# simonsobs/hmvec

Hardware: AMD Instinct MI355X
Metric: (z,m,k) grid-points/sec for P_1h+P_2h (higher is better)
Workload: dtype f64

## Files before the change

### hmvec_amd/_native.py

```python
import ctypes as C
import math
import os

import numpy as np

_HERE = os.path.dirname(os.path.abspath(__file__))
LIB_PATH = os.environ.get("HMG_LIB_PATH") or os.path.join(_HERE, "libhmgrid.so")
ABI_VERSION = 10
COMM_ID_BYTES = 128

c_double_p = C.c_void_p


class NativeError(RuntimeError):
    pass


class HaloStageArgs(C.Structure):
    _fields_ = [("d_zs", C.c_void_p), ("d_delta", C.c_void_p), ("d_rho", C.c_void_p),
                ("duffy_A", C.c_double), ("duffy_alpha", C.c_double), ("duffy_beta", C.c_double),
                ("h", C.c_double), ("d_cs", C.c_void_p), ("d_rvir", C.c_void_p), ("d_rs", C.c_void_p),
                ("d_nfw_series", C.c_void_p), ("d_drho1", C.c_void_p), ("delta2", C.c_double),
                ("d_rho2", C.c_void_p), ("d_m2", C.c_void_p), ("d_r2", C.c_void_p)]

# ... 109 lines not shown
    "hmg_sigma2_massfn": [_P, _I, _I, _I, _P, _P, _P, _P, _D, C.POINTER(MassFnParams), _P, _P, _P, _P, _P, _P],
    "hmg_sigma2_massfn_halo": [_P, _I, _I, _I, _P, _P, _P, _P, _D, C.POINTER(MassFnParams), _P, _P, _P, _P, _P, _P,
                               C.POINTER(HaloStageArgs)],
    "hmg_halo_stage": [_P, _I, _I, _P, _P, _P, _P, _D, _D, _D, _D, _P, _P, _P, _P, _P, _D, _P, _P, _P],
    "hmg_massfn": [_P, _I, _I, C.POINTER(MassFnParams), _P, _P, _P, _P, _P, _P],
    "hmg_halo_structure": [_P, _I, _I, _P, _P, _P, _P, _D, _D, _D, _D, _P, _P, _P],
    "hmg_mdelta_convert": [_P, _I, _I, _P, _P, _P, _D, _P, _P, _P],
    "hmg_nfw_analytic": [_P, _I, _I, _I, _P, _P, _P, _P, _P, _P],
    "hmg_profile_rowparams": [_P, _I, _I, _I, _P, _P, _P, _P, _P, _P, C.POINTER(_D * 9), _D, _D, _D,
                              _D, _P, _P, _P, _P, _P, _P, _P],
    "hmg_profile_rows_from_mvir": [_P, _I, _I, _I, _P, _P, _P, _P, _P, _D, _P, _P, C.POINTER(_D * 9), _D, _D,
                                   _D, _D, _P, _P, _P, _P, _P, _P, _P, _P, _P],
    "hmg_profile_fft": [_P, _I, _I, _I, _I, _D, _P, _P, _P, _P, _P, _P, _D, _D, _D, _D, _D,
                        _P, _P, _P, _P, _I, _P, _P, _P, _P, _P],
    "hmg_profile_fft_logx": [_P, _I, _P, _P],
    "hmg_hod": [_P, _I, _I, C.POINTER(HodParams), _P, _P, _P, _P, _P, _P, _P, _P, _P, _P, _P, _P],
    "hmg_power": [_P, _I, _I, _I, C.POINTER(Tracer), C.POINTER(Tracer), _P, _P, _P, _P, _P, _P,
                  _D, _D, _P, _P],
    "hmg_power_batch": [_P, _I, _I, _I, _I, C.POINTER(Tracer), _I, C.POINTER(_I), C.POINTER(_I),
                        _P, _P, _P, _P, _P, _P, _D, _D, C.POINTER(_P), C.POINTER(_P)],
    "hmg_power_2halo_terms": [_P, _I, _I, _I, C.POINTER(Tracer), C.POINTER(Tracer), _P, _P, _P, _P, _P, _D,
                              _P, _P, _P],
    "hmg_sigma2_halo_front": [_P, _I, _I, _I, _P, _P, _P, _P, _D, _P, C.POINTER(HaloStageArgs), C.POINTER(HodPart),
                              C.POINTER(RowsPart)],
    "hmg_group_rows": [_P, _I, _I, _I, _I, C.POINTER(MassFnPart), C.POINTER(HodPart), C.POINTER(RowsPart),
                       C.POINTER(NfwPart)],
    "hmg_group_profile": [_P, _I, _I, _I, C.POINTER(ProfileFftPart), C.POINTER(HodPart), C.POINTER(PowerBatchDesc)],
    "hmg_group_tensors": [_P, _I, _I, _I, _I, C.POINTER(MassFnPart), C.POINTER(HodPart), C.POINTER(PowerBatchDesc),
                          C.POINTER(NfwPart), C.POINTER(ProfileFftPart)],
    "hmg_power_batch_run": [_P, _I, _I, _I, C.POINTER(PowerBatchDesc), _I],
# ... 219 lines not shown
        self.call_now("hmg_event_record", slot)

    def lane(self, i):
        self.flush()
        self.call_now("hmg_lane_set", i)

    def wait(self, slot):
        self.flush()
        self.call_now("hmg_event_wait", slot)

    def elapsed_ms(self, s0, s1):
        ms = C.c_double()
        check(self.lib.hmg_elapsed_ms(self.handle, s0, s1, C.byref(ms)))
        return ms.value

    _NO_FLUSH = frozenset(["hmg_bracket_next", "hmg_profile_support_epoch"])

    def call(self, name, *args):
        if name not in self._NO_FLUSH:
            self.flush()
        if self._trace is not None:
            self._trace.append((name, args))
        check(getattr(self.lib, name)(self.handle, *args))

    def capture(self, fn):
        self.flush()
        check(self.lib.hmg_graph_begin(self.handle))
        self.capture_serial += 1
        try:
            fn()
            self.flush()
# ... 57 lines not shown
```

### hmvec_amd/csrc/hmctx.hpp

```cpp
#pragma once
#include <hip/hip_runtime.h>
#include <rccl/rccl.h>
#include <rocfft/rocfft.h>

#include <cstdio>
#include <map>
#include <string>
#include <tuple>
#include <vector>

#include "../../include/hmgrid.h"
#include "ldsfft.hpp"
#include "sici.hpp"

extern thread_local std::string g_last_error;
int fail(const char* what, const char* detail, const char* file, int line);
#define HIP_TRY(expr)                                                                   \
    do {                                                                                \
        hipError_t e_ = (expr);                                                         \
        if (e_ != hipSuccess) {                                                         \
            (void)hipGetLastError();                                                    \
            return fail(#expr, hipGetErrorString(e_), __FILE__, __LINE__);              \
        }                                                                               \
    } while (0)
// ... 38 lines not shown
    hmg::UnpackTw* twNr = nullptr;
};
struct ChirpPlan {
    hmg::cplx *chP = nullptr, *chJ = nullptr, *Bw = nullptr;
    int Jw = 0;
};
struct SupportKey {
    const void *cmax, *xs, *rss, *ks;
    int rows, nxs, nk;
    long long epoch;
    bool operator<(const SupportKey& o) const {
        return std::tie(cmax, xs, rss, ks, rows, nxs, nk, epoch) < std::tie(o.cmax, o.xs, o.rss, o.ks, o.rows, o.nxs, o.nk, o.epoch);
    }
};

struct hmg_ctx {
    int device = 0;
    hipStream_t stream = nullptr;
    hipStream_t lanes[HMG_LANES] = {};
    int lane = 0;
    hipEvent_t ev[HMG_EVENT_SLOTS] = {};
    int bracket[HMG_KERNEL_COUNT][2];
    void* scratch[7] = {nullptr, nullptr, nullptr, nullptr, nullptr, nullptr, nullptr};
    size_t scratch_bytes[7] = {0, 0, 0, 0, 0, 0, 0};
    std::map<std::pair<int, int>, FftPlan> plans;
    std::map<int, struct FusedPlan> fused;
    size_t fft_chunk_bytes = 0;
    int use_fused_fft = 1;
    int use_pruned_fft = 1;
    int fused_max_m = 6144;
// ... 22 lines not shown
    char* up_ring = nullptr;
    hipEvent_t up_ev[UP_SLOTS] = {};
    int up_next = 0;
    hipEvent_t pin_ev[2] = {nullptr, nullptr};
    int num_cu = 256;
    std::multimap<size_t, void*> free_blocks;
    std::map<void*, size_t> block_bytes;
    size_t cached_bytes = 0;
    bool lanes_dirty = false;
    bool capturing = false;
    std::vector<void*> freed_in_capture;
    std::map<int, std::vector<void*>> graph_blocks;
    std::map<int, hipGraphExec_t> graphs;
    std::map<int, int> graph_kernels;
    int next_graph_id = 1;
    hmg_ctx() { for (auto& b : bracket) b[0] = b[1] = -1; }
};
constexpr size_t FREE_CACHE_LIMIT = (size_t)4 << 30;

int event_at(hmg_ctx* c, int slot, hipEvent_t* out);
int check_fault(hmg_ctx* c);
int sync_all(hmg_ctx* c);
int ensure_scratch(hmg_ctx* c, int slot, size_t bytes);
int bracket_open(hmg_ctx* c, int kid, int* stop_slot);
int bracket_close(hmg_ctx* c, int stop_slot);
static inline dim3 grid1d(size_t n, int block) { return dim3((unsigned)((n + block - 1) / block)); }
```

### hmvec_amd/csrc/hmgrid.hip

```cpp
#include <algorithm>
#include <cmath>
#include <cstdlib>
#include <cstring>

#include "hmctx.hpp"
#include "fastmath.hpp"
#include "rowdev.hpp"
#include "longgrid.hpp"

#include "kernels/common.hpp"
#include "kernels/sigma2.hpp"
#include "kernels/massfn.hpp"
#include "kernels/halo.hpp"
#include "kernels/nfw.hpp"
#include "kernels/rows.hpp"
#include "kernels/profile_chain.hpp"
#include "kernels/profile_fused.hpp"
#include "kernels/hod.hpp"
#include "kernels/power.hpp"
#include "kernels/power_batch.hpp"
#include "kernels/groups.hpp"
#include "kernels/limber.hpp"
#include "kernels/functions.hpp"

// ... 594 lines not shown
    A.nconst = p.d_nconst; A.cconst = p.d_cconst;
    A.logx = p.d_logxs;
    A.rho_tab = R.rho_tab; A.rho_shared = R.rho_shared;
    A.rowsc = (p.d_rowsc && p.d_nconst) ? p.d_rowsc : nullptr;
    return A;
}

static int profile_fft_impl(hmg_ctx* c, int nz, int nm, int nk, const hmg_profile_fft_part& p, FftRiders& R) {
    const int nxs = p.nxs;
    const double step = p.fft_step;
    const double *xs = p.d_xs, *kts = p.d_kts, *cmax = p.d_cmax, *rss = p.d_rss, *zs = p.d_zs, *ks = p.d_ks;
    R.chain_done = R.nfw_done = false;
    REQUIRE(c && xs && kts && cmax && rss && zs && ks && p.d_out, "NULL argument");
    REQUIRE((p.d_nconst == nullptr) == (p.d_cconst == nullptr), "pass both hint arrays or neither");
    REQUIRE(nz > 0 && nm > 0 && nk > 0, "empty grid");
    REQUIRE(nxs >= 4, "nxs too small");
    const int nh = nxs / 2;
    const int rows = nz * nm;
    REQUIRE(step > 0.0, "step must be positive");
    const bool table = R.rho_tab != nullptr;
    FftRoute r;
    if (fft_route(c, p, R.C && R.nchain > 0, table, &r)) return 1;
    if (r.try_long) {
        int took = 0;
        if (profile_fft_pruned(c, fused_args(nm, nk, p, nullptr, R), rows, r.FP != nullptr, &took)) return 1;
        if (took) return 0;
    }
    if (r.FP) {
        FusedArgs A = fused_args(nm, nk, p, r.FP, R);
        int stop = -1;
        if (bracket_open(c, HMG_KERNEL_PROFILE_FFT, &stop)) return 1;
        if (!table && !A.logx && rows >= 8192) {
            if (ensure_scratch(c, 2, (size_t)nxs * 8)) return 1;
            hipLaunchKernelGGL(logx_kernel, grid1d((size_t)nxs, 256), dim3(256), 0, c->stream, nxs, xs,
                               (double*)c->scratch[2]);
            HIP_TRY(hipGetLastError());
            A.logx = (const double*)c->scratch[2];
        }
        int rc;
        if (table) rc = with_shape(r.shape, [&](auto s) { return launch_table<decltype(s)>(c, A, rows); });
        else if (r.grouped) rc = with_shape(r.shape, [&](auto s) { return launch_group<decltype(s)>(c, A, rows, R); });
        else rc = with_shape(r.shape, [&](auto s) { return launch_fused<decltype(s)>(c, A, rows); });
        if (rc) return 1;
        R.chain_done = r.grouped;
        R.nfw_done = r.grouped && R.N;
        return bracket_close(c, stop);
    }
    const size_t per_row = (size_t)nxs * 8 + (size_t)(nh + 1) * 16;
    size_t budget = c->fft_chunk_bytes ? c->fft_chunk_bytes : ((size_t)160 << 20);
    int chunk = (int)(budget / per_row);
    if (chunk < 1) chunk = 1;
    if (chunk > rows) chunk = rows;
    if (ensure_scratch(c, 0, (size_t)chunk * nxs * 8)) return 1;
    if (ensure_scratch(c, 1, (size_t)chunk * (nh + 1) * 16)) return 1;
    if (ensure_scratch(c, 2, (size_t)chunk * 8)) return 1;
    double* fin = (double*)c->scratch[0];
    double2* fout = (double2*)c->scratch[1];
    double* mnorm = (double*)c->scratch[2];
// ... 28 lines not shown
    return bracket_close(c, stop);
}

int hmg_profile_fft(hmg_ctx* c, int nz, int nm, int nk, int nxs, double step, const double* xs, const double* kts,
                    const double* amp, const double* xcs, const double* alpha, const double* expo,
                    double amp_c, double xc_c, double alpha_c, double expo_c, double gamma,
                    const double* cmax, const double* rss, const double* zs, const double* ks,
                    int do_mass_norm, const double* post, double* out, int* nconst, double* cconst,
                    const double* logxs) {
    const hmg_profile_fft_part p{nxs, step, xs, kts, amp, xcs, alpha, expo, amp_c, xc_c, alpha_c, expo_c, gamma,
                                 cmax, rss, zs, ks, do_mass_norm, post, out, nconst, cconst, logxs};
    FftRiders R;
    return profile_fft_impl(c, nz, nm, nk, p, R);
}

int hmg_profile_support_epoch(hmg_ctx* c, long long epoch) {
    REQUIRE(c, "NULL ctx");
    c->support_epoch = epoch;
    return 0;
}

int hmg_profile_fft_logx(hmg_ctx* c, int nxs, const double* xs, double* logxs) {
    REQUIRE(c && xs && logxs && nxs > 0, "bad argument");
    hipLaunchKernelGGL(logx_kernel, grid1d((size_t)nxs, 256), dim3(256), 0, c->stream, nxs, xs, logxs);
    HIP_TRY(hipGetLastError());
    return 0;
}

int hmg_hod(hmg_ctx* c, int nz, int nm, const hmg_hod_params* p, const double* zs, const double* ms,
            const double* lthr, const double* nzm, const double* bh, const double* wm, double* Nc,
// ... 620 lines not shown
```

### hmvec_amd/csrc/kernels/power_batch.hpp

```cpp
#pragma once

namespace hmg {

constexpr int PB_MAXTR = 4;
constexpr int PB_MAXPAIR = PB_MAXTR * (PB_MAXTR + 1) / 2;

constexpr unsigned PB_LIN(int s) { return 1u | ((unsigned)s << 2); }
constexpr unsigned PB_HOD(int s) { return 2u | ((unsigned)s << 2); }
constexpr unsigned pb_code(unsigned t0, unsigned t1 = 0, unsigned t2 = 0, unsigned t3 = 0) {
    return t0 | (t1 << 4) | (t2 << 8) | (t3 << 12);
}
constexpr int pb_kind(unsigned code, int r) { return (int)((code >> (4 * r)) & 3u); }
constexpr int pb_slot(unsigned code, int r) { return (int)((code >> (4 * r + 2)) & 3u); }
constexpr int pb_ncoef(unsigned code, int ntr) {
    int n = 2;
    for (int r = 0; r < ntr; ++r) n += pb_kind(code, r) == 2 ? 4 : 1;
    return n;
}
constexpr int pb_stride(unsigned code, int ntr, int nc1) {
    return code ? ((pb_ncoef(code, ntr) + 7) & ~7) : 2 + ntr * 3 * nc1;
}

#define PB_SPEC_LIST                                                  \
    PB_SPEC(1, 1, PB_LIN(0))                                          \
// ... 157 lines not shown
    double kstar;
    int nm, nk;
};

constexpr int PB_NV = 16;

__device__ __forceinline__ double lane_value(double v, int l) {
    const int lo = __builtin_amdgcn_readlane(__double2loint(v), l), hi = __builtin_amdgcn_readlane(__double2hiint(v), l);
    return __hiloint2double(hi, lo);
}

template <int NT, int NTR, int V, bool W16, unsigned CODE = 0>
__global__ __launch_bounds__(W16 ? 1024 : 512) void power_batch_kernel(BatchArgs A) {
    extern __shared__ double red[];
    using vec_t = typename VecT<V>::type;
    constexpr int NC1 = 1 + NT;
    constexpr int STRIDE = pb_stride(CODE, NTR, NC1);
    constexpr int NPAIR = NTR * (NTR + 1) / 2;
    constexpr int NACC = NTR + NPAIR;
    const int lane = threadIdx.x & 63;
    const int wv = __builtin_amdgcn_readfirstlane(threadIdx.x >> 6);
    const int z = blockIdx.y;
    const int k0 = (blockIdx.x * 64 + lane) * V;
    const bool live = k0 < A.nk;
    double acc[NACC][V];
#pragma unroll
    for (int a = 0; a < NACC; ++a)
#pragma unroll
        for (int v = 0; v < V; ++v) acc[a][v] = 0.0;
    const size_t zrow = (size_t)z * A.nm;
// ... 204 lines not shown
```

### hmvec_amd/csrc/kernels/profile_fused.hpp

```cpp
#pragma once

namespace hmg {


__global__ void logx_kernel(int n, const double* __restrict__ xs, double* __restrict__ out) {
    const int i = blockIdx.x * blockDim.x + threadIdx.x;
    if (i < n) out[i] = log_fast(xs[i]);
}


template <int NT, int R, int MAXB, bool SMALL = false, int NIN = R, int SRC_SHIFT = 0>
__device__ __forceinline__ void fused_pass(cplx* buf, const cplx* __restrict__ twM, int M, int Ns, int twstep,
                                           unsigned magic, int keep) {
    cplx v[MAXB][R];
    const int nb = M / R;
#pragma unroll
    for (int b = 0; b < MAXB; ++b) {
        const int j = threadIdx.x + b * NT;
        if (j < nb && (keep < 0 || j <= keep || j >= nb - keep)) pass_load<R, SMALL, NIN, SRC_SHIFT>(buf, twM, M, Ns, twstep, magic, j, v[b]);
    }
    __syncthreads();
#pragma unroll
    for (int b = 0; b < MAXB; ++b) {
        const int j = threadIdx.x + b * NT;
// ... 162 lines not shown
        if (j <= half && (j <= jn || hi)) {
            u[j - 1] = ua[b];
            if (hi && M - j >= 1) u[M - j - 1] = ub[b];
        }
    }
    if (threadIdx.x == 0) u[M - 1] = 0.0;
    __syncthreads();
    const double k_lo = RSC ? rsc[1] : red[20], k_hi = RSC ? rsc[2] : red[21], inv_dk = RSC ? rsc[3] : red[22];
    const double pf = A.post ? A.post[row] : 1.0;
    const double u1 = u[0];
    double* __restrict__ dst = A.out + (size_t)row * A.nk;
    const int nleft = RSC ? __double2loint(rsc[5]) : (A.nconst ? __builtin_amdgcn_readfirstlane(*s_cnt) : 0);
    if (nleft > 0) {
        typedef double v2d __attribute__((ext_vector_type(2)));
        const double c = u1 * pf;
        const int head = (int)((reinterpret_cast<uintptr_t>(dst) >> 3) & 1);
        const int npair = (nleft - head) >> 1;
        v2d* __restrict__ d2 = reinterpret_cast<v2d*>(dst + head);
        const v2d cc = {c, c};
        for (int q = threadIdx.x; q < npair; q += NT) __builtin_nontemporal_store(cc, &d2[q]);
        if (threadIdx.x == 0) {
            if (head) __builtin_nontemporal_store(c, &dst[0]);
            if ((nleft - head) & 1) __builtin_nontemporal_store(c, &dst[nleft - 1]);
        }
    }
    auto interp = [&](double k) {
        int j = (int)(k * inv_dk);
        j = j < 1 ? 1 : (j > M - 1 ? M - 1 : j);
        const double fr = fma(k, inv_dk, -(double)j);
        const double y0 = u[j - 1], y1 = u[j];
        return fma(y1 - y0, fr, y0);
    };
    if (A.nconst) {
        for (int i = (nleft & ~63) + threadIdx.x; i < A.nk; i += NT) {
            if (i < nleft) continue;
            const double k = A.ks[i];
            const double val = k > k_hi ? 0.0 : interp(k);
            __builtin_nontemporal_store(val * pf, &dst[i]);
// ... 9 lines not shown
        A.nconst[row] = nleft;
        A.cconst[row] = u1 * pf;
    }
}
template <int NT, int MAXB, int MAXP, int SPECM>
__global__ __launch_bounds__(NT, (fused_occ<MAXB, SPECM>())) void profile_fused_kernel(FusedArgs A) {
    extern __shared__ __attribute__((aligned(16))) double smem[];
    profile_fused_row<NT, MAXB, MAXP, SPECM>(A, blockIdx.x, smem);
}
template <int NT, int MAXB, int MAXP, int SPECM>
__global__ __launch_bounds__(NT, (fused_occ<MAXB, SPECM>())) void profile_table_kernel(FusedArgs A) {
    extern __shared__ __attribute__((aligned(16))) double smem[];
    profile_fused_row<NT, MAXB, MAXP, SPECM, true>(A, blockIdx.x, smem);
}


}
```

### hmvec_amd/csrc/rowdev.hpp

```cpp
#pragma once
#include <hip/hip_runtime.h>

#include "fastmath.hpp"
#include "ldsfft.hpp"

#ifndef HMG_FUSED_NT
#define HMG_FUSED_NT 512
#endif

namespace hmg {

constexpr int FUSED_NT = HMG_FUSED_NT;

constexpr int WAVE = 64;

template <int CTRL, int ROW_MASK>
__device__ __forceinline__ double dpp_move(double v) {
    const int lo = __builtin_amdgcn_update_dpp(0, __double2loint(v), CTRL, ROW_MASK, 0xf, false);
    const int hi = __builtin_amdgcn_update_dpp(0, __double2hiint(v), CTRL, ROW_MASK, 0xf, false);
    return __hiloint2double(hi, lo);
}
__device__ __forceinline__ double wave_sum(double v) {
    v += dpp_move<0xB1, 0xf>(v);
    v += dpp_move<0x4E, 0xf>(v);
// ... 9 lines not shown
    FftPlanDev plan;
    int nxs, nm, nk, do_norm;
    const double* xs;
    const cplx* twM;
    const UnpackTw* twN;
    const double* kts;
    const double *amp, *xc, *alpha, *expo;
    double amp_c, xc_c, alpha_c, expo_c, gamma, step;
    const double *cmax, *rss, *zs, *ks, *post;
    double* out;
    int* nconst;
    double* cconst;
    const double* logx;
    const double* rho_tab;
    int rho_shared;
    const double* rowsc;
};

__device__ __forceinline__ double gnfw_rho_fast(double lt , double A, double AL, double EX,
                                                double gamma) {
    const double ta = exp_fast<false>(fmin(AL * lt, 700.0));
    return A * exp_fast<false>(gamma * lt - EX * log1p_abs(ta));
}

__device__ __forceinline__ double gnfw_rho_alpha1(double lt , double t , double A, double EX,
                                                  double gamma) {
    return A * exp_fast<false>(gamma * lt - EX * log1p_abs(t));
}

}
// ... 1 lines not shown
```

### hmvec_amd/csrc/runtime.hip

```cpp
#include <algorithm>
#include <cmath>
#include <cstdlib>
#include <cstring>

#include "hmctx.hpp"

using namespace hmg;

thread_local std::string g_last_error;

int fail(const char* what, const char* detail, const char* file, int line) {
    char buf[512];
    snprintf(buf, sizeof(buf), "%s: %s (%s:%d)", what, detail, file, line);
    g_last_error = buf;
    return 1;
}

static int rocfft_refcount = 0;

int event_at(hmg_ctx* c, int slot, hipEvent_t* out) {
    if (!c->ev[slot]) HIP_TRY(hipEventCreate(&c->ev[slot]));
    *out = c->ev[slot];
    return 0;
}
// ... 158 lines not shown
    HIP_TRY(e);
    c->block_bytes[*d_out] = bytes;
    return 0;
}
int hmg_free(hmg_ctx* c, void* p) {
    REQUIRE(c, "NULL ctx");
    if (!p) return 0;
    auto it = c->block_bytes.find(p);
    REQUIRE(it != c->block_bytes.end(), "pointer was not allocated by hmg_malloc of this context");
    if (c->capturing) {
        c->freed_in_capture.push_back(p);
        return 0;
    }
    if (c->lanes_dirty && sync_all(c)) return 1;
    const size_t bytes = it->second;
    if (c->cached_bytes + bytes <= FREE_CACHE_LIMIT) {
        c->free_blocks.emplace(bytes, p);
        c->cached_bytes += bytes;
        return 0;
    }
    if (sync_all(c)) return 1;
    HIP_TRY(hipFree(p));
    c->block_bytes.erase(it);
    return 0;
}
int hmg_host_alloc(hmg_ctx* c, size_t bytes, void** h_out) {
    REQUIRE(c && h_out, "NULL argument");
    HIP_TRY(hipSetDevice(c->device));
    HIP_TRY(hipHostMalloc(h_out, bytes ? bytes : 8, hipHostMallocDefault));
    return 0;
// ... 160 lines not shown
    int nkern = 0;
    {
        size_t nn = 0;
        if (hipGraphGetNodes(g, nullptr, &nn) == hipSuccess && nn) {
            std::vector<hipGraphNode_t> nodes(nn);
            if (hipGraphGetNodes(g, nodes.data(), &nn) == hipSuccess)
                for (size_t i = 0; i < nn; ++i) {
                    hipGraphNodeType t;
                    if (hipGraphNodeGetType(nodes[i], &t) == hipSuccess && t == hipGraphNodeTypeKernel) ++nkern;
                }
        }
    }
    hipGraphExec_t ge = nullptr;
    hipError_t e = hipGraphInstantiate(&ge, g, nullptr, nullptr, 0);
    (void)hipGraphDestroy(g);
    if (e != hipSuccess) release_deferred_frees(c);
    HIP_TRY(e);
    *id = c->next_graph_id++;
    c->graphs[*id] = ge;
    c->graph_kernels[*id] = nkern;
    c->graph_blocks[*id].swap(c->freed_in_capture);
    return 0;
}
int hmg_graph_kernel_nodes(hmg_ctx* c, int id, int* n) {
    REQUIRE(c && n, "NULL argument");
    auto it = c->graph_kernels.find(id);
    REQUIRE(it != c->graph_kernels.end(), "unknown graph id");
    *n = it->second;
    return 0;
}
int hmg_graph_abort(hmg_ctx* c) {
    REQUIRE(c, "NULL ctx");
    if (!c->capturing) return 0;
    c->capturing = false;
    release_deferred_frees(c);
    c->lane = 0;
    c->stream = c->lanes[0];
    hipGraph_t g = nullptr;
    (void)hipStreamEndCapture(c->lanes[0], &g);
    if (g) (void)hipGraphDestroy(g);
    (void)hipGetLastError();
    return 0;
}
int hmg_graph_launch(hmg_ctx* c, int id) {
    REQUIRE(c, "NULL ctx");
    REQUIRE(!c->capturing, "cannot replay a graph inside a capture");
    auto it = c->graphs.find(id);
    REQUIRE(it != c->graphs.end(), "unknown graph id");
    HIP_TRY(hipGraphLaunch(it->second, c->stream));
    return 0;
}
int hmg_graph_destroy(hmg_ctx* c, int id) {
    REQUIRE(c, "NULL ctx");
    auto it = c->graphs.find(id);
    if (it == c->graphs.end()) return 0;
    if (sync_all(c)) return 1;
    HIP_TRY(hipGraphExecDestroy(it->second));
    c->graphs.erase(it);
    auto gb = c->graph_blocks.find(id);
    if (gb != c->graph_blocks.end()) {
        for (void* p : gb->second) (void)hmg_free(c, p);
        c->graph_blocks.erase(gb);
    }
    return 0;
}

int hmg_bracket_next(hmg_ctx* c, int kernel_id, int s0, int s1) {
    REQUIRE(c && kernel_id >= 0 && kernel_id < HMG_KERNEL_COUNT, "bad kernel id");
    REQUIRE(s0 >= -1 && s0 < HMG_EVENT_SLOTS && s1 >= -1 && s1 < HMG_EVENT_SLOTS, "bad event slot");
    c->bracket[kernel_id][0] = s0;
    c->bracket[kernel_id][1] = s1;
    return 0;
}
// ... 22 lines not shown
```

### hmvec_amd/halomodel.py

```python
import ctypes as C
import itertools
import os
from collections.abc import MutableMapping

import numpy as np
import scipy.constants as constants

from . import _native as nat
from .cosmology import Cosmology, _is_shared_product, sigma2_kgrid, sigma2_weights
from .params import battaglia_defaults, default_params
from .quadrature import gradient_is_uniform, simpson_weights, trapz_weights
from .functions import FN_BG_INTEGRAND, FN_ST_FSIGMA, FN_TINKER_FSIGMA, fn2d, ngal_from_mthresh, trapz_lastaxis
from .functions import context as fn_context
from .utils import vectorized_bisection_search

_trapz = getattr(np, "trapezoid", None) or np.trapz
_EPOCHS = itertools.count(1)
_DATA = os.path.join(os.path.dirname(os.path.abspath(__file__)), "data")


def _tinker_alpha_table():
    with np.load(os.path.join(_DATA, "tinker10_alpha_of_z.npz")) as f:
        return f["z"], f["alpha"]


class DeviceDict(MutableMapping):

    def __init__(self, ctx_getter, on_change=None):
        self._ctx_getter = ctx_getter
        self._on_change = on_change or (lambda: None)
        self._dev = {}
        self._host = {}
        self._hint = {}

    def dev(self, name):
        return self._dev[name]

    def hint(self, name):
        return self._hint.get(name, (None, None))

    def set_dev(self, name, darr, hint=None):
        self._dev[name] = darr
        self._host.pop(name, None)
        if hint is None:
            self._hint.pop(name, None)
        else:
            self._hint[name] = hint
        self._on_change()

    def __getitem__(self, name):
        if name not in self._host:
            self._host[name] = self._dev[name].numpy()
        return self._host[name]

    def __setitem__(self, name, value):
        if isinstance(value, nat.DeviceArray):
            self.set_dev(name, value)
        else:
            self.set_dev(name, self._ctx_getter().upload(np.asarray(value, dtype=np.float64)))

    def __delitem__(self, name):
        del self._dev[name]
        self._host.pop(name, None)
        self._hint.pop(name, None)
        self._on_change()

    def __contains__(self, name):
# ... 48 lines not shown
        self.zs = np.asarray(zs, dtype=np.float64)
        self.ks = np.asarray(ks, dtype=np.float64)
        self._device = device
        self.ctx = ctx
        Cosmology.__init__(self, params, halofit, engine=engine, accuracy=accuracy, background=background)

        self.mdef = mdef
        self.mode = mass_function
        self.hods = {}
        self._dcache = {}
        self._pool = {}
        self._use_lanes = os.environ.get("HMG_LANES", "0") == "1"
        self._groups = os.environ.get("HMG_NO_GROUPS", "0") != "1" and not self._use_lanes
        self._stages = []
        self._stage_dims = None

        self._pcache = {}
        self._version = 0
        self.uk_profiles = DeviceDict(self._ctx, self._bump)
        self.pk_profiles = DeviceDict(self._ctx, self._bump)

        if ms is not None:
            self.ms = np.asarray(ms, dtype=np.float64)
            self.init_mass_function(self.ms)

        if not skip_nfw:
            self.add_nfw_profile("nfw", numeric=nfw_numeric)

    def _init_cosmology(self, params, halofit):
        Cosmology._init_cosmology(self, params, halofit)
# ... 147 lines not shown
            occ = None
            if "hod" in st:
                occ = nat.HodPart.from_buffer_copy(st["hod"])
                occ.stage, st["hod"].stage = nat.HOD_OCCUPATIONS, nat.HOD_SUMS
                hod_sums = True
            args = st.pop("front")
            rows = st.pop("rows") if "rows" in st and "rows_alone" not in x else None
            ctx.call_now("hmg_sigma2_halo_front", *args[:-1], C.byref(args[-1]), C.byref(occ) if occ is not None else None,
                         C.byref(rows) if rows is not None else None)
        elif "hod" in st:
            h = st.pop("hod")
            ctx.call_now("hmg_hod", nz, nm, h.h_par, h.d_zs, h.d_ms, h.d_log10mstar_thresh, h.d_nzm, h.d_bh, h.d_wm,
                         h.d_Nc, h.d_Ns, h.d_NsNsm1, h.d_NcNs, h.d_ngal, h.d_bg)
        if "fft" in st and ("massfn" in st or "nfw" in st) and "rows" not in st and not x:
            ctx.call_now("hmg_profile_support_epoch", getattr(self, "_epoch", 0))
            try:
                ctx.call_now("hmg_group_tensors", nz, nm, nk, nq, ref("massfn"), ref("hod") if hod_sums else None,
                             C.byref(prep) if prep is not None else None, ref("nfw"), ref("fft"))
            finally:
                ctx.call_now("hmg_profile_support_epoch", 0)
            return prep is not None
        nfw_alone = st.pop("nfw") if "nfw_alone" in x and "nfw" in st else None
        if any(k in st for k in ("massfn", "rows", "nfw")):
            ctx.call_now("hmg_group_rows", nz, nm, nk, nq, ref("massfn"), None, ref("rows"), ref("nfw"))
        if nfw_alone is not None:
            ctx.call_now("hmg_nfw_analytic", nz, nm, nk, nfw_alone.d_cs, nfw_alone.d_rs, nfw_alone.d_zs, nfw_alone.d_ks,
                         nfw_alone.d_nfw_series, nfw_alone.d_uk)
        if "fft" in st or hod_sums:
            if "chain_alone" in x and "fft" in st and (hod_sums or prep is not None):
                ctx.call_now("hmg_group_profile", nz, nm, nk, None, ref("hod") if hod_sums else None,
                             C.byref(prep) if prep is not None else None)
                ctx.call_now("hmg_group_profile", nz, nm, nk, ref("fft"), None, None)
                return prep is not None
            ctx.call_now("hmg_profile_support_epoch", getattr(self, "_epoch", 0))
            try:
                ctx.call_now("hmg_group_profile", nz, nm, nk, ref("fft"), ref("hod") if hod_sums else None,
                             C.byref(prep) if prep is not None else None)
            finally:
                ctx.call_now("hmg_profile_support_epoch", 0)
            return prep is not None
        return False

    def get_sigma2(self):
        return self.sigma2

    def _tinker_z_params(self):
        zs = self.zs
        zc = zs * np.heaviside(3 - zs, 0) + 3 * np.heaviside(zs - 3, 0)
        tz, ta = _tinker_alpha_table()
        if np.any(zc < tz[0]) or np.any(zc > tz[-1]):
            raise ValueError("A value in x_new is outside the interpolation range.")
        alpha = np.interp(zc, tz, ta)
        beta = 0.589 * (1 + zc) ** 0.20
# ... 157 lines not shown
        hint = None
        if self._dcache["ks_ascending"]:
            hint = (self._buf((key, "nconst"), ((nz * nm + 1) // 2,)), self._buf((key, "cconst"), (nz, nm)))
        amp, xc, alpha, expo = rowp
        args = (int(nxs), step, d_xs.ptr, d_kts.ptr,
                nat.ptr(amp), nat.ptr(xc), nat.ptr(alpha), nat.ptr(expo),
                float(consts[0]), float(consts[1]), float(consts[2]), float(consts[3]), float(gamma),
                d_cmax.ptr, d_rss.ptr, self._d_zs().ptr, self._d_ks().ptr, int(do_mass_norm),
                nat.ptr(d_post), out.ptr, nat.ptr(hint[0] if hint else None), nat.ptr(hint[1] if hint else None),
                d_lx.ptr)
        if self._groups:
            self._queue("fft", nat.ProfileFftPart(*args, nat.ptr(d_rowsc if hint else None)))
        else:
            ctx.flush()
            ctx.call("hmg_profile_support_epoch", getattr(self, "_epoch", 0))
            try:
                ctx.call("hmg_profile_fft", nz, nm, nk, *args)
            finally:
                ctx.call("hmg_profile_support_epoch", 0)
        return out, hint

    def _battaglia_rowparams(self, key, kind, fit9, gamma, alpha_const, pref, post_pref, nxs=None, xmax=None):
        ctx = self._ctx()
        nz, nm = self._nz, self._nm
        outs = [self._buf((key, "rowp", i), (nz, nm)) for i in range(7)]
        fit = (C.c_double * 9)(*fit9)
        d_hz = self._dev("hz", lambda: self.h_of_z(self.zs))
        d_rhoc = self._dev("rhocz", lambda: self.rho_critical_z(self.zs))
        if not getattr(self, "_m200c_valid", False):
            m2, r2 = self._buf("m200c", (nz, nm)), self._buf("r200c", (nz, nm))
            ctx.call("hmg_profile_rows_from_mvir", kind, nz, nm, self._d_ms().ptr, self._d_cs.ptr,
                     self._d_rvir.ptr, self._d_zs().ptr, self._d_drho1().ptr, 200.0, d_rhoc.ptr, d_hz.ptr,
                     C.byref(fit), float(gamma), float(alpha_const), float(pref), float(post_pref),
# ... 191 lines not shown

        return vectorized_bisection_search(ngal, ngal_of,
                                           [pparams["hod_bisection_search_min_log10mthresh"],
                                            pparams["hod_bisection_search_max_log10mthresh"]],
                                           "decreasing", rtol=pparams["hod_bisection_search_rtol"], verbose=True,
                                           hang_check_num_iter=pparams["hod_bisection_search_warn_iter"])

    def get_ngal(self, Nc, Ns):
        with fn_context(self._ctx()):
            return ngal_from_mthresh(nzm=self.nzm, ms=self.ms, Ncs=Nc, Nss=Ns)

    def get_bg(self, Nc, Ns, ngal):
        with fn_context(self._ctx()):
            return trapz_lastaxis(fn2d(FN_BG_INTEGRAND, [self.nzm, Nc, Ns, self.bh]), self.ms) / ngal

    def _tracer(self, name, order):
        def tensor(dd, nm_):
            d_ = dd.dev(nm_)
            if tuple(d_.shape) != (self._nz, self._nm, self._nk):
                raise ValueError(f"profile {nm_!r} has shape {tuple(d_.shape)}, the model's grid is "
                                 f"{(self._nz, self._nm, self._nk)}")
            return d_
        for kind in order:
            if kind == "h" and name in self.hods:
                hod = self.hods[name]
                cn = hod["central_profile"]
                d = hod.dev
                sn = hod["satellite_profile"]
                hs = self.uk_profiles.hint(sn)
                hc = self.uk_profiles.hint(cn) if cn is not None else (None, None)
                t = nat.Tracer(nat.TRACER_HOD, tensor(self.uk_profiles, sn).ptr,
                               None if cn is None else tensor(self.uk_profiles, cn).ptr,
                               d["Nc"].ptr, d["Ns"].ptr, d["NcNs"].ptr, d["NsNsm1"].ptr, d["ngal"].ptr, None,
# ... 17 lines not shown
        ctx.call("hmg_power", nz, nm, nk, C.byref(ta), C.byref(tb), self._d_nzm.ptr, self._d_bh.ptr,
                 self._d_ms().ptr, self._d_wm().ptr, self._d_ks().ptr, self._d_Pzk().ptr,
                 self._rho_m0(), float(self.p["kstar_damping"]), nat.ptr(d1), nat.ptr(d2))
        self._sync_point()
        return d1, d2

    def _rho_m0(self):
        if getattr(self, "_rho_m0_val", None) is None:
            self._rho_m0_val = float(self.rho_matter_z(0)[0])
        return self._rho_m0_val

    def power_device(self, name, name2=None, b1_in=None, b2_in=None, want=("1h", "2h"), out1=None, out2=None):
        name2 = name if name2 is None else name2
        keep = []
        want1, want2 = "1h" in want, "2h" in want
        a1, ka1 = self._tracer(name, "hmp")
        b1, kb1 = self._tracer(name2, "hmp")
        a2, ka2 = self._tracer(name, "mph") if want2 else (a1, ka1)
        b2, kb2 = self._tracer(name2, "mph") if want2 else (b1, kb1)
        if want2:
            if b1_in is not None:
                keep.append(self._ctx().upload(np.asarray(b1_in, dtype=np.float64).reshape(-1)))
                a2.d_bias_override = keep[-1].ptr
            if b2_in is not None:
                n = b1_in.shape[0]
                keep.append(self._ctx().upload(np.asarray(b2_in, dtype=np.float64).reshape((n, 1))))
                b2.d_bias_override = keep[-1].ptr
        same = (ka1 == ka2) and (kb1 == kb2)
        if want1 and want2 and same:
            d1, d2 = self._power_launch(a2, b2, True, True, out1, out2)
# ... 1 lines not shown
            d1 = self._power_launch(a1, b1, True, False, out1, None)[0] if want1 else None
            d2 = self._power_launch(a2, b2, False, True, None, out2)[1] if want2 else None
        if keep:
            self._ctx().sync()
        return d1, d2

    def power_device_batch(self, pairs, outs1=None, outs2=None):
        ctx = self._ctx()
        nz, nm, nk = self._nz, self._nm, self._nk
        pairs = [(a, a if b is None else b) for a, b in pairs]
        names = []
        for a, b in pairs:
            for n_ in (a, b):
                if n_ not in names:
                    names.append(n_)
        res1 = [self._tracer(n_, "hmp") for n_ in names]
        res2 = [self._tracer(n_, "mph") for n_ in names]
        kinds = {n_: r[1] for n_, r in zip(names, res1)}
        batchable = len(names) <= 4 and all(r1[1] == r2[1] for r1, r2 in zip(res1, res2))
        batchable = batchable and not any(a != b and kinds[a] == kinds[b] and kinds[a] in "hp"
                                          for a, b in pairs)
        o1 = [outs1[i] if outs1 is not None else ctx.empty((nz, nk)) for i in range(len(pairs))]
        o2 = [outs2[i] if outs2 is not None else ctx.empty((nz, nk)) for i in range(len(pairs))]
        if not batchable:
            for i, (a, b) in enumerate(pairs):
                self.power_device(a, b, out1=o1[i], out2=o2[i])
            return o1, o2
        uniq, alias = [], []
        for a, b in pairs:
            key = tuple(sorted((names.index(a), names.index(b))))
            if key not in uniq:
                uniq.append(key)
# ... 27 lines not shown
        for a, b in pairs:
            for nm_ in (a, a if b is None else b):
                if nm_ not in seen:
                    seen.append(nm_)
        self._tsz_notice(*seen)
        o1, o2 = self.power_device_batch(pairs)
        return {tuple(p): self._sum_on_device(a, b) for p, a, b in zip(pairs, o1, o2)}

    def _tsz_notice(self, *names):
        for nm_ in names:
            if nm_ not in self.uk_profiles and nm_ in self.pk_profiles:
                print("Check the consistency relation for tSZ")

    def _tensor_names(self, nm_):
        try:
            k1, k2 = self._tracer(nm_, "hmp")[1], self._tracer(nm_, "mph")[1]
        except (ValueError, KeyError):
            return None
        if k1 != k2:
            return None
        if k1 == "h":
            hod = self.hods[nm_]
            return {("uk", hod["satellite_profile"])} | (
                {("uk", hod["central_profile"])} if hod["central_profile"] is not None else set())
        return {("uk" if k1 == "m" else "pk", nm_)}

    _SMALL_GRID_BYTES = 32 << 20

    def _tensors_valid(self, tn):
        shape = (self._nz, self._nm, self._nk)
        for kind, nm_ in tn:
# ... 6 lines not shown
        need = self._tensor_names(name)
        need2 = self._tensor_names(name2)
        if need is None or need2 is None:
            return None
        need = need | need2
        kinds = {}
        names = [name] + ([name2] if name2 != name else [])
        small = self._nz * self._nm * self._nk * 8 <= self._SMALL_GRID_BYTES
        for cand in list(self.hods) + list(self.uk_profiles) + list(self.pk_profiles):
            if cand in names or len(names) >= 4:
                continue
            tn = self._tensor_names(cand)
            if tn is not None and (tn <= need or small) and self._tensors_valid(tn):
                names.append(cand)
        for n_ in names:
            kinds[n_] = self._tracer(n_, "hmp")[1]
        pairs = []
        for i, a in enumerate(names):
            for b in names[i:]:
                if a != b and kinds[a] == kinds[b] and kinds[a] in "hp":
                    continue
                pairs.append((a, b))
        return pairs

    def _power_cached(self, name, name2):
        name2 = name if name2 is None else name2
        ent = self._pcache.get((name, name2))
        if ent is not None and ent[0] == self._version:
            return ent[1], ent[2]
        pairs = self._free_riders(name, name2)
        if pairs and ((name, name2) in pairs or (name2, name) in pairs):
# ... 274 lines not shown
```

### include/hmgrid.h

```cpp
#ifndef HMGRID_H
#define HMGRID_H

#include <stddef.h>

#ifdef __cplusplus
extern "C" {
#endif

#define HMG_ABI_VERSION 10

typedef struct hmg_ctx hmg_ctx;

int         hmg_abi_version(void);
const char* hmg_last_error(void);
int hmg_ctx_create(int device, hmg_ctx** out);
int hmg_ctx_destroy(hmg_ctx* ctx);
int hmg_malloc(hmg_ctx* ctx, size_t bytes, void** d_out);
int hmg_free(hmg_ctx* ctx, void* d_ptr);
int hmg_memcpy_h2d(hmg_ctx* ctx, void* d_dst, const void* h_src, size_t bytes);
int hmg_memcpy_d2h(hmg_ctx* ctx, void* h_dst, const void* d_src, size_t bytes);
int hmg_memcpy_d2d(hmg_ctx* ctx, void* d_dst, const void* d_src, size_t bytes);
int hmg_sync(hmg_ctx* ctx);
int hmg_host_alloc(hmg_ctx* ctx, size_t bytes, void** h_out);
int hmg_host_free(hmg_ctx* ctx, void* h_ptr);
// ... 109 lines not shown

int hmg_profile_fft(hmg_ctx* ctx, int nz, int nm, int nk, int nxs, double fft_step,
                    const double* d_xs, const double* d_kts,
                    const double* d_amp, const double* d_xc, const double* d_alpha,
                    const double* d_expo, double amp_const, double xc_const,
                    double alpha_const, double expo_const, double gamma,
                    const double* d_cmax , const double* d_rss ,
                    const double* d_zs, const double* d_ks, int do_mass_norm,
                    const double* d_post ,
                    double* d_out ,
                    int* d_nconst , double* d_cconst ,
                    const double* d_logxs );
int hmg_profile_support_epoch(hmg_ctx* ctx, long long epoch);
int hmg_profile_fft_logx(hmg_ctx* ctx, int nxs, const double* d_xs, double* d_logxs);

typedef struct {
    double sig_log_mstellar, alphasat, Bsat, betasat, Bcut, betacut;
    int    corr;
} hmg_hod_params;
int hmg_hod(hmg_ctx* ctx, int nz, int nm, const hmg_hod_params* h_par, const double* d_zs,
            const double* d_ms, const double* d_log10mstar_thresh ,
            const double* d_nzm, const double* d_bh, const double* d_wm ,
            double* d_Nc, double* d_Ns, double* d_NsNsm1, double* d_NcNs ,
            double* d_ngal , double* d_bg );

#define HMG_TRACER_MATTER   0
#define HMG_TRACER_HOD      1
#define HMG_TRACER_PRESSURE 2
typedef struct {
    int kind;
// ... 194 lines not shown
```

Baseline: 822.4 billion.

## Defer writing constant low-k prefix of profile rows until a consumer needs it

```diff
diff --git a/hmvec_amd/_native.py b/hmvec_amd/_native.py
--- a/hmvec_amd/_native.py
+++ b/hmvec_amd/_native.py
@@ -147,6 +147,10 @@
     "hmg_profile_fft": [_P, _I, _I, _I, _I, _D, _P, _P, _P, _P, _P, _P, _D, _D, _D, _D, _D,
                         _P, _P, _P, _P, _I, _P, _P, _P, _P, _P],
     "hmg_profile_fft_logx": [_P, _I, _P, _P],
+    "hmg_prefix_deferral": [_P, _I],
+    "hmg_prefix_fill": [_P, _P],
+    "hmg_prefix_pending": [_P, _P, C.POINTER(_I)],
+    "hmg_prefix_fill_rows": [_P, _P, _P, _P, _I, _I],
     "hmg_hod": [_P, _I, _I, C.POINTER(HodParams), _P, _P, _P, _P, _P, _P, _P, _P, _P, _P, _P, _P],
     "hmg_power": [_P, _I, _I, _I, C.POINTER(Tracer), C.POINTER(Tracer), _P, _P, _P, _P, _P, _P,
                   _D, _D, _P, _P],
@@ -396,7 +400,7 @@
         check(self.lib.hmg_elapsed_ms(self.handle, s0, s1, C.byref(ms)))
         return ms.value
 
-    _NO_FLUSH = frozenset(["hmg_bracket_next", "hmg_profile_support_epoch"])
+    _NO_FLUSH = frozenset(["hmg_bracket_next", "hmg_profile_support_epoch", "hmg_prefix_deferral"])
 
     def call(self, name, *args):
         if name not in self._NO_FLUSH:
diff --git a/hmvec_amd/csrc/hmctx.hpp b/hmvec_amd/csrc/hmctx.hpp
--- a/hmvec_amd/csrc/hmctx.hpp
+++ b/hmvec_amd/csrc/hmctx.hpp
@@ -76,6 +76,13 @@
     }
 };
 
+struct PrefixEntry {
+    int* nconst = nullptr;
+    double* cconst = nullptr;
+    int rows = 0, nk = 0;
+    bool pending = false;
+};
+
 struct hmg_ctx {
     int device = 0;
     hipStream_t stream = nullptr;
@@ -128,6 +135,10 @@
     std::map<int, hipGraphExec_t> graphs;
     std::map<int, int> graph_kernels;
     int next_graph_id = 1;
+    int prefix_deferral = 0;
+    std::map<void*, PrefixEntry> prefix;
+    std::map<void*, PrefixEntry> prefix_capture;
+    std::map<int, std::map<void*, PrefixEntry>> graph_prefix;
     hmg_ctx() { for (auto& b : bracket) b[0] = b[1] = -1; }
 };
 constexpr size_t FREE_CACHE_LIMIT = (size_t)4 << 30;
@@ -138,4 +149,19 @@
 int ensure_scratch(hmg_ctx* c, int slot, size_t bytes);
 int bracket_open(hmg_ctx* c, int kid, int* stop_slot);
 int bracket_close(hmg_ctx* c, int stop_slot);
+static inline void prefix_note(hmg_ctx* c, void* out, const PrefixEntry& e) {
+    auto& m = c->capturing ? c->prefix_capture : c->prefix;
+    if (e.nconst || c->capturing) m[out] = e;
+    else m.erase(out);
+}
+static inline void prefix_replayed(hmg_ctx* c, const std::map<void*, PrefixEntry>& fx) {
+    for (auto& kv : fx) {
+        if (kv.second.nconst) c->prefix[kv.first] = kv.second;
+        else c->prefix.erase(kv.first);
+    }
+}
+static inline void prefix_drop_block(hmg_ctx* c, void* p, size_t bytes) {
+    auto lo = c->prefix.lower_bound(p), hi = c->prefix.lower_bound((char*)p + bytes);
+    c->prefix.erase(lo, hi);
+}
 static inline dim3 grid1d(size_t n, int block) { return dim3((unsigned)((n + block - 1) / block)); }
diff --git a/hmvec_amd/csrc/hmgrid.hip b/hmvec_amd/csrc/hmgrid.hip
--- a/hmvec_amd/csrc/hmgrid.hip
+++ b/hmvec_amd/csrc/hmgrid.hip
@@ -632,6 +632,7 @@
     REQUIRE(c && xs && kts && cmax && rss && zs && ks && p.d_out, "NULL argument");
     REQUIRE((p.d_nconst == nullptr) == (p.d_cconst == nullptr), "pass both hint arrays or neither");
     REQUIRE(nz > 0 && nm > 0 && nk > 0, "empty grid");
+    prefix_note(c, p.d_out, PrefixEntry{p.d_nconst, p.d_cconst, nz * nm, nk, false});
     REQUIRE(nxs >= 4, "nxs too small");
     const int nh = nxs / 2;
     const int rows = nz * nm;
@@ -646,6 +647,7 @@
     }
     if (r.FP) {
         FusedArgs A = fused_args(nm, nk, p, r.FP, R);
+        A.defer = c->prefix_deferral && A.nconst;
         int stop = -1;
         if (bracket_open(c, HMG_KERNEL_PROFILE_FFT, &stop)) return 1;
         if (!table && !A.logx && rows >= 8192) {
@@ -660,6 +662,7 @@
         else if (r.grouped) rc = with_shape(r.shape, [&](auto s) { return launch_group<decltype(s)>(c, A, rows, R); });
         else rc = with_shape(r.shape, [&](auto s) { return launch_fused<decltype(s)>(c, A, rows); });
         if (rc) return 1;
+        if (A.defer) prefix_note(c, p.d_out, PrefixEntry{A.nconst, A.cconst, rows, nk, true});
         R.chain_done = r.grouped;
         R.nfw_done = r.grouped && R.N;
         return bracket_close(c, stop);
@@ -718,6 +721,52 @@
     return profile_fft_impl(c, nz, nm, nk, p, R);
 }
 
+int hmg_prefix_deferral(hmg_ctx* c, int on) {
+    REQUIRE(c, "NULL ctx");
+    c->prefix_deferral = on != 0;
+    return 0;
+}
+
+int hmg_prefix_fill_rows(hmg_ctx* c, double* out, const int* nconst, const double* cconst, int rows, int nk) {
+    REQUIRE(c && out && nconst && cconst, "NULL argument");
+    REQUIRE(rows > 0 && nk > 0, "empty grid");
+    hipLaunchKernelGGL(prefix_fill_kernel, dim3(rows), dim3(256), 0, c->stream, nk, nconst, cconst, out);
+    HIP_TRY(hipGetLastError());
+    return 0;
+}
+
+int hmg_prefix_pending(hmg_ctx* c, const double* out, int* pending) {
+    REQUIRE(c && out && pending, "NULL argument");
+    REQUIRE(!c->capturing, "the pending state is what replays make it: ask outside the captured step");
+    auto it = c->prefix.find((void*)out);
+    *pending = it != c->prefix.end() && it->second.pending;
+    return 0;
+}
+
+int hmg_prefix_fill(hmg_ctx* c, double* out) {
+    REQUIRE(c && out, "NULL argument");
+    PrefixEntry e;
+    if (c->capturing) {
+        auto ic = c->prefix_capture.find(out);
+        if (ic != c->prefix_capture.end()) {
+            if (!ic->second.nconst || !ic->second.pending) return 0;
+            e = ic->second;
+        } else {
+            auto ig = c->prefix.find(out);
+            if (ig == c->prefix.end()) return 0;
+            e = ig->second;
+        }
+    } else {
+        auto it = c->prefix.find(out);
+        if (it == c->prefix.end() || !it->second.pending) return 0;
+        e = it->second;
+    }
+    if (hmg_prefix_fill_rows(c, out, e.nconst, e.cconst, e.rows, e.nk)) return 1;
+    e.pending = false;
+    prefix_note(c, out, e);
+    return 0;
+}
+
 int hmg_profile_support_epoch(hmg_ctx* c, long long epoch) {
     REQUIRE(c, "NULL ctx");
     c->support_epoch = epoch;
diff --git a/hmvec_amd/csrc/kernels/power_batch.hpp b/hmvec_amd/csrc/kernels/power_batch.hpp
--- a/hmvec_amd/csrc/kernels/power_batch.hpp
+++ b/hmvec_amd/csrc/kernels/power_batch.hpp
@@ -195,6 +195,8 @@
 __global__ __launch_bounds__(W16 ? 1024 : 512) void power_batch_kernel(BatchArgs A) {
     extern __shared__ double red[];
     using vec_t = typename VecT<V>::type;
+    static_assert(V == 1 || V == 2, "k-tile widths the deferred left fill was checked for");
+    static_assert(HMG_PREFIX_TILE % (64 * V) == 0, "HMG_PREFIX_TILE must be a multiple of every k-tile width");
     constexpr int NC1 = 1 + NT;
     constexpr int STRIDE = pb_stride(CODE, NTR, NC1);
     constexpr int NPAIR = NTR * (NTR + 1) / 2;
diff --git a/hmvec_amd/csrc/kernels/profile_fused.hpp b/hmvec_amd/csrc/kernels/profile_fused.hpp
--- a/hmvec_amd/csrc/kernels/profile_fused.hpp
+++ b/hmvec_amd/csrc/kernels/profile_fused.hpp
@@ -200,14 +200,17 @@
     if (nleft > 0) {
         typedef double v2d __attribute__((ext_vector_type(2)));
         const double c = u1 * pf;
-        const int head = (int)((reinterpret_cast<uintptr_t>(dst) >> 3) & 1);
-        const int npair = (nleft - head) >> 1;
-        v2d* __restrict__ d2 = reinterpret_cast<v2d*>(dst + head);
+        const int nskip = A.defer ? (nleft & ~(HMG_PREFIX_TILE - 1)) : 0;
+        double* __restrict__ d0 = dst + nskip;
+        const int nfill = nleft - nskip;
+        const int head = (int)((reinterpret_cast<uintptr_t>(d0) >> 3) & 1);
+        const int npair = (nfill - head) >> 1;
+        v2d* __restrict__ d2 = reinterpret_cast<v2d*>(d0 + head);
         const v2d cc = {c, c};
         for (int q = threadIdx.x; q < npair; q += NT) __builtin_nontemporal_store(cc, &d2[q]);
-        if (threadIdx.x == 0) {
-            if (head) __builtin_nontemporal_store(c, &dst[0]);
-            if ((nleft - head) & 1) __builtin_nontemporal_store(c, &dst[nleft - 1]);
+        if (threadIdx.x == 0 && nfill > 0) {
+            if (head) __builtin_nontemporal_store(c, &d0[0]);
+            if ((nfill - head) & 1) __builtin_nontemporal_store(c, &d0[nfill - 1]);
         }
     }
     auto interp = [&](double k) {
@@ -247,5 +250,25 @@
     profile_fused_row<NT, MAXB, MAXP, SPECM, true>(A, blockIdx.x, smem);
 }
 
-
-}
+__global__ __launch_bounds__(256) void prefix_fill_kernel(int nk, const int* __restrict__ nconst,
+                                                          const double* __restrict__ cconst, double* __restrict__ out) {
+    typedef double v2d __attribute__((ext_vector_type(2)));
+    const int row = blockIdx.x;
+    int n = nconst[row] & ~(HMG_PREFIX_TILE - 1);
+    n = n < nk ? n : nk;
+    if (n <= 0) return;
+    const double c = cconst[row];
+    double* __restrict__ dst = out + (size_t)row * nk;
+    const int head = (int)((reinterpret_cast<uintptr_t>(dst) >> 3) & 1);
+    const int npair = (n - head) >> 1;
+    v2d* __restrict__ d2 = reinterpret_cast<v2d*>(dst + head);
+    const v2d cc = {c, c};
+    for (int q = threadIdx.x; q < npair; q += 256) __builtin_nontemporal_store(cc, &d2[q]);
+    if (threadIdx.x == 0) {
+        if (head) __builtin_nontemporal_store(c, &dst[0]);
+        if ((n - head) & 1) __builtin_nontemporal_store(c, &dst[n - 1]);
+    }
+}
+
+
+}
diff --git a/hmvec_amd/csrc/rowdev.hpp b/hmvec_amd/csrc/rowdev.hpp
--- a/hmvec_amd/csrc/rowdev.hpp
+++ b/hmvec_amd/csrc/rowdev.hpp
@@ -47,6 +47,7 @@
     const double* logx;
     const double* rho_tab;
     int rho_shared;
+    int defer;
     const double* rowsc;
 };
 
diff --git a/hmvec_amd/csrc/runtime.hip b/hmvec_amd/csrc/runtime.hip
--- a/hmvec_amd/csrc/runtime.hip
+++ b/hmvec_amd/csrc/runtime.hip
@@ -196,6 +196,7 @@
     }
     if (c->lanes_dirty && sync_all(c)) return 1;
     const size_t bytes = it->second;
+    prefix_drop_block(c, p, bytes);
     if (c->cached_bytes + bytes <= FREE_CACHE_LIMIT) {
         c->free_blocks.emplace(bytes, p);
         c->cached_bytes += bytes;
@@ -386,12 +387,14 @@
     hipGraphExec_t ge = nullptr;
     hipError_t e = hipGraphInstantiate(&ge, g, nullptr, nullptr, 0);
     (void)hipGraphDestroy(g);
-    if (e != hipSuccess) release_deferred_frees(c);
+    if (e != hipSuccess) { release_deferred_frees(c); c->prefix_capture.clear(); }
     HIP_TRY(e);
     *id = c->next_graph_id++;
     c->graphs[*id] = ge;
     c->graph_kernels[*id] = nkern;
     c->graph_blocks[*id].swap(c->freed_in_capture);
+    c->graph_prefix[*id].swap(c->prefix_capture);
+    c->prefix_capture.clear();
     return 0;
 }
 int hmg_graph_kernel_nodes(hmg_ctx* c, int id, int* n) {
@@ -406,6 +409,7 @@
     if (!c->capturing) return 0;
     c->capturing = false;
     release_deferred_frees(c);
+    c->prefix_capture.clear();
     c->lane = 0;
     c->stream = c->lanes[0];
     hipGraph_t g = nullptr;
@@ -420,6 +424,8 @@
     auto it = c->graphs.find(id);
     REQUIRE(it != c->graphs.end(), "unknown graph id");
     HIP_TRY(hipGraphLaunch(it->second, c->stream));
+    auto gp = c->graph_prefix.find(id);
+    if (gp != c->graph_prefix.end()) prefix_replayed(c, gp->second);
     return 0;
 }
 int hmg_graph_destroy(hmg_ctx* c, int id) {
@@ -429,6 +435,7 @@
     if (sync_all(c)) return 1;
     HIP_TRY(hipGraphExecDestroy(it->second));
     c->graphs.erase(it);
+    c->graph_prefix.erase(id);
     auto gb = c->graph_blocks.find(id);
     if (gb != c->graph_blocks.end()) {
         for (void* p : gb->second) (void)hmg_free(c, p);
diff --git a/hmvec_amd/halomodel.py b/hmvec_amd/halomodel.py
--- a/hmvec_amd/halomodel.py
+++ b/hmvec_amd/halomodel.py
@@ -33,8 +33,19 @@
         self._host = {}
         self._hint = {}
 
-    def dev(self, name):
-        return self._dev[name]
+    def dev(self, name, fill=True):
+        d = self._dev[name]
+        if fill and name in self._hint:
+            self._ctx_getter().call("hmg_prefix_fill", d.ptr)
+        return d
+
+    def _pending(self, name):
+        if name not in self._hint:
+            return False
+        ctx = self._ctx_getter()
+        n = C.c_int()
+        nat.check(ctx.lib.hmg_prefix_pending(ctx.handle, self._dev[name].ptr, C.byref(n)))
+        return bool(n.value)
 
     def hint(self, name):
         return self._hint.get(name, (None, None))
@@ -49,8 +60,10 @@
         self._on_change()
 
     def __getitem__(self, name):
+        if name in self._host and self._pending(name):
+            del self._host[name]
         if name not in self._host:
-            self._host[name] = self._dev[name].numpy()
+            self._host[name] = self.dev(name).numpy()
         return self._host[name]
 
     def __setitem__(self, name, value):
@@ -129,6 +142,7 @@
         self._groups = os.environ.get("HMG_NO_GROUPS", "0") != "1" and not self._use_lanes
         self._stages = []
         self._stage_dims = None
+        self.prefix_deferral = os.environ.get("HMG_NO_PREFIX_DEFERRAL", "0") != "1"
 
         self._pcache = {}
         self._version = 0
@@ -306,10 +320,12 @@
                          h.d_Nc, h.d_Ns, h.d_NsNsm1, h.d_NcNs, h.d_ngal, h.d_bg)
         if "fft" in st and ("massfn" in st or "nfw" in st) and "rows" not in st and not x:
             ctx.call_now("hmg_profile_support_epoch", getattr(self, "_epoch", 0))
+            ctx.call_now("hmg_prefix_deferral", int(self.prefix_deferral))
             try:
                 ctx.call_now("hmg_group_tensors", nz, nm, nk, nq, ref("massfn"), ref("hod") if hod_sums else None,
                              C.byref(prep) if prep is not None else None, ref("nfw"), ref("fft"))
             finally:
+                ctx.call_now("hmg_prefix_deferral", 0)
                 ctx.call_now("hmg_profile_support_epoch", 0)
             return prep is not None
         nfw_alone = st.pop("nfw") if "nfw_alone" in x and "nfw" in st else None
@@ -325,10 +341,12 @@
                 ctx.call_now("hmg_group_profile", nz, nm, nk, ref("fft"), None, None)
                 return prep is not None
             ctx.call_now("hmg_profile_support_epoch", getattr(self, "_epoch", 0))
+            ctx.call_now("hmg_prefix_deferral", int(self.prefix_deferral))
             try:
                 ctx.call_now("hmg_group_profile", nz, nm, nk, ref("fft"), ref("hod") if hod_sums else None,
                              C.byref(prep) if prep is not None else None)
             finally:
+                ctx.call_now("hmg_prefix_deferral", 0)
                 ctx.call_now("hmg_profile_support_epoch", 0)
             return prep is not None
         return False
@@ -516,9 +534,11 @@
         else:
             ctx.flush()
             ctx.call("hmg_profile_support_epoch", getattr(self, "_epoch", 0))
+            ctx.call("hmg_prefix_deferral", int(self.prefix_deferral))
             try:
                 ctx.call("hmg_profile_fft", nz, nm, nk, *args)
             finally:
+                ctx.call("hmg_prefix_deferral", 0)
                 ctx.call("hmg_profile_support_epoch", 0)
         return out, hint
 
@@ -740,9 +760,9 @@
         with fn_context(self._ctx()):
             return trapz_lastaxis(fn2d(FN_BG_INTEGRAND, [self.nzm, Nc, Ns, self.bh]), self.ms) / ngal
 
-    def _tracer(self, name, order):
+    def _tracer(self, name, order, fill=True):
         def tensor(dd, nm_):
-            d_ = dd.dev(nm_)
+            d_ = dd.dev(nm_, fill=fill)
             if tuple(d_.shape) != (self._nz, self._nm, self._nk):
                 raise ValueError(f"profile {nm_!r} has shape {tuple(d_.shape)}, the model's grid is "
                                  f"{(self._nz, self._nm, self._nk)}")
@@ -790,6 +810,7 @@
         name2 = name if name2 is None else name2
         keep = []
         want1, want2 = "1h" in want, "2h" in want
+        self._main()
         a1, ka1 = self._tracer(name, "hmp")
         b1, kb1 = self._tracer(name2, "hmp")
         a2, ka2 = self._tracer(name, "mph") if want2 else (a1, ka1)
@@ -821,8 +842,8 @@
             for n_ in (a, b):
                 if n_ not in names:
                     names.append(n_)
-        res1 = [self._tracer(n_, "hmp") for n_ in names]
-        res2 = [self._tracer(n_, "mph") for n_ in names]
+        res1 = [self._tracer(n_, "hmp", fill=False) for n_ in names]
+        res2 = [self._tracer(n_, "mph", fill=False) for n_ in names]
         kinds = {n_: r[1] for n_, r in zip(names, res1)}
         batchable = len(names) <= 4 and all(r1[1] == r2[1] for r1, r2 in zip(res1, res2))
         batchable = batchable and not any(a != b and kinds[a] == kinds[b] and kinds[a] in "hp"
@@ -880,7 +901,7 @@
 
     def _tensor_names(self, nm_):
         try:
-            k1, k2 = self._tracer(nm_, "hmp")[1], self._tracer(nm_, "mph")[1]
+            k1, k2 = self._tracer(nm_, "hmp", fill=False)[1], self._tracer(nm_, "mph", fill=False)[1]
         except (ValueError, KeyError):
             return None
         if k1 != k2:
@@ -917,7 +938,7 @@
             if tn is not None and (tn <= need or small) and self._tensors_valid(tn):
                 names.append(cand)
         for n_ in names:
-            kinds[n_] = self._tracer(n_, "hmp")[1]
+            kinds[n_] = self._tracer(n_, "hmp", fill=False)[1]
         pairs = []
         for i, a in enumerate(names):
             for b in names[i:]:
diff --git a/include/hmgrid.h b/include/hmgrid.h
--- a/include/hmgrid.h
+++ b/include/hmgrid.h
@@ -147,6 +147,12 @@
 int hmg_profile_support_epoch(hmg_ctx* ctx, long long epoch);
 int hmg_profile_fft_logx(hmg_ctx* ctx, int nxs, const double* d_xs, double* d_logxs);
 
+#define HMG_PREFIX_TILE 128
+int hmg_prefix_deferral(hmg_ctx* ctx, int on);
+int hmg_prefix_fill(hmg_ctx* ctx, double* d_out);
+int hmg_prefix_pending(hmg_ctx* ctx, const double* d_out, int* pending);
+int hmg_prefix_fill_rows(hmg_ctx* ctx, double* d_out, const int* d_nconst, const double* d_cconst, int rows, int nk);
+
 typedef struct {
     double sig_log_mstellar, alphasat, Bsat, betasat, Bcut, betacut;
     int    corr;
```

Result: faster. 857.9 billion (median of 6 runs) (+4.3%).
